# wells-wood-research/timed-design

Measured on AMD Instinct MI355X. Metric: residue_frames_per_sec, higher is better.
Workload: dtype f32

## Files before the change

timed-design_amd/csrc/common.h:

```cpp
#pragma once
#include <hip/hip_runtime.h>
#include <stdint.h>
#include <string>
#include <vector>

#include "../../include/timed_hip.h"

enum : int {
    OP_INPUT = 0, OP_CONV3D, OP_DENSE, OP_BN, OP_ACT, OP_MAXPOOL, OP_AVGPOOL, OP_GAP, OP_GMP,
    OP_FLATTEN, OP_CONCAT, OP_ADD, OP_IDENTITY
};
enum : int { ACT_LINEAR = 0, ACT_RELU, ACT_ELU, ACT_SOFTMAX, ACT_SIGMOID, ACT_TANH, ACT_LEAKY };

void th_set_error(const char* fmt, ...);
#define TH_FAIL(code, ...)          \
    do {                            \
        th_set_error(__VA_ARGS__);  \
        return (code);              \
    } while (0)
#define HIP_TRY(expr)                                                                            \
    do {                                                                                         \
        hipError_t _e = (expr);                                                                  \
        if (_e != hipSuccess) {                                                                  \
            th_set_error("%s failed: %s (%s:%d)", #expr, hipGetErrorString(_e), __FILE__, __LINE__); \
            return TH_EHIP;                                                                      \
        }                                                                                        \
    } while (0)

#ifndef TH_KNOCKOUTS
#define TH_KNOCKOUTS 0
#endif
#if TH_KNOCKOUTS
#define TH_KNOCK_FIELD int dbg;
#define TH_KNOCK(a) ((a).dbg)
#define TH_KNOCK_SET(a, v) ((a).dbg = (v))
#else
#define TH_KNOCK_FIELD
#define TH_KNOCK(a) 0
#define TH_KNOCK_SET(a, v) ((void)0)
#endif

struct ThKnobs {
    int winograd = 1;
    int wino_split = 1;
    int wfused = 1;
    int wf_split = 1;
    int lanes = 1, lane_lag = 1;
    int guard = 1;
    int first_wino = 1;
    int first_split = 1;
    int conv_gl = 1;
    int dense_gemm = 1;
    int first_int = 1;
    int no_pool_first = 0;
    int no_tail_fuse = 0;
    int conv_notail = 0, n16_resident = 0;
    int wf_resident = 0, wf_noblk = 0;
    long long wino_piece = 0;
    int wino_b3var = 2, wino_nomid = 0;
#if TH_KNOCKOUTS
    int wf_dbg = 0, first_dbg = 0, wino_dbg = 0, conv_dbg = 0, pw_dbg = 0;
#endif
    std::string nondefault;
};
int th_knobs_read(ThKnobs* k);
inline const ThKnobs& th_knobs_of(const ThKnobs* k) { static const ThKnobs dflt; return k ? *k : dflt; }

hipError_t th_malloc_retry_impl(void** p, size_t bytes);
template <class T> inline hipError_t th_malloc_retry(T** p, size_t bytes) { return th_malloc_retry_impl(reinterpret_cast<void**>(p), bytes); }

int th_usable_cpus();

struct TView {
    float* p = nullptr;
    int D = 1, H = 1, W = 1, C = 0;
    int cs = 0;
    int coff = 0;
    int64_t fs = 0;
    int blk = 0;
    int V() const { return D * H * W; }
};

#define TH_MAX_POST 4
enum : int { POP_ACT = 1, POP_AFFINE = 2 };
struct PostOps {
    int n = 0;
    int type[TH_MAX_POST] = {0, 0, 0, 0};
    int act[TH_MAX_POST] = {0, 0, 0, 0};
    float alpha[TH_MAX_POST] = {0, 0, 0, 0};
    const float* scale[TH_MAX_POST] = {nullptr, nullptr, nullptr, nullptr};
    const float* shift[TH_MAX_POST] = {nullptr, nullptr, nullptr, nullptr};
    int monotone = 0;
};
struct PreOp {
    const float* scale = nullptr;
    const float* shift = nullptr;
    int act = ACT_LINEAR;
    float alpha = 0.f;
};

struct ConvGeom {
    int kd, kh, kw, sd, sh, sw, dd, dh, dw;
    int pz, py, px;
};
int launch_convert_frames(hipStream_t s, const void* src, int dtype, int64_t n, int V, int C, TView dst);
int launch_conv3d_direct(hipStream_t s, int64_t n, TView in, TView out, ConvGeom g, const float* w, const float* bias,
                         PreOp pre, PostOps post);
int launch_pool3d(hipStream_t s, int64_t n, TView in, TView out, ConvGeom g, int is_max);
int launch_eltwise(hipStream_t s, int64_t n, TView in, TView out, PostOps ops);
int launch_global_pool(hipStream_t s, int64_t n, TView in, TView out, int is_max);
int launch_dense(hipStream_t s, int64_t n, TView in, TView out, const float* w, const float* bias, PostOps post);
inline bool conv_gl_wanted(int knob, const ConvGeom& g, int Vo) { return knob == 2 || (knob == 1 && (g.sd > 1 || g.sh > 1 || g.sw > 1 || Vo <= 64)); }
bool conv_gl_ok(int Cin, int Cout, int in_cs, int in_coff, int64_t in_fs);
size_t conv_gl_wpk_floats(const ConvGeom& g, int Cin, int Cout);
double conv_gl_exec_flops(const ConvGeom& g, int Cin, int Cout, int Vo);
std::string conv_gl_label(int Cout);
void conv_gl_pack_weights(const ConvGeom& g, int Cin, int Cout, const float* w, float* dst);
int launch_conv_gl(hipStream_t s, int64_t n, TView in, TView out, ConvGeom g, int Cin, int Cout, const float* wpk, const float* bias, PreOp pre, PostOps post);
bool dense_gemm_ok(int F, int O, int64_t xfs);
int launch_dense_gemm(hipStream_t s, int64_t n, TView in, TView out, const float* w, const float* bias, PostOps post);
int launch_softmax(hipStream_t s, int64_t n, TView in, TView out);
int launch_gap_softmax(hipStream_t s, int64_t n, TView in, TView logits, TView probs);
int launch_tail_dense(hipStream_t s, int64_t n, TView in, PostOps pre, TView pooled, TView logits, TView probs, const float* w,
                      const float* bias, PostOps post, int softmax);
int launch_copy(hipStream_t s, int64_t n, TView in, TView out);
int launch_add(hipStream_t s, int64_t n, TView a, TView b, TView out);
int launch_synth_frames(hipStream_t s, float* d, int64_t n, int side, int channels, int atoms, uint64_t seed);

struct ConvMfmaPlan {
    int cfg = -1;
    int CI = 0, CS = 0;
    int BN = 0;
    int nnb = 0;
    int nchunks = 0;
    int pool = 0;
    int Dc = 0, Hc = 0, Wc = 0;
    int FB = 1, ZB = 0, nzb = 1;
    int Zp = 0, Hp = 0, Wp = 0;
    int rows_pf = 0;
    size_t lds_bytes = 0;
    size_t tab_off = 0;
    size_t wpk_floats = 0;
// ... 148 lines not shown
```

timed-design_amd/csrc/conv_wino.hip:

```cpp
#include "bf16x3.h"
#include "common.h"
#include "device_math.h"
#include "wino_tables.h"

#include <algorithm>
#include <cstdlib>
#include <cstring>
#include <thread>
#include <vector>

namespace {

constexpr int kZ = WINO_N;
constexpr int kNF = 64;
constexpr int kKC = 32;
constexpr int kCB = 128;

template <int R, int C>
__device__ __forceinline__ void wino_apply(const float (&T)[R][C], const float (&in)[C], float (&out)[R]) {
#pragma unroll
    for (int r = 0; r < R; ++r) {
        float acc = 0.f;
        bool first = true;
#pragma unroll
// ... 92 lines not shown

template <int kP, bool GAP = false>
__global__ void __launch_bounds__(256) k_wino_out(const WinoOutArgs a) {
    constexpr int kPos = kP * kP;
    const unsigned idx = blockIdx.x * 256u + threadIdx.x;
    const unsigned co = idx % (unsigned)a.Cout, f = idx / (unsigned)a.Cout;
    if (f >= (unsigned)a.n) return;
    const unsigned ioff = f * (unsigned)a.Coutp + co;
    const unsigned ooff = f * (unsigned)a.out_fs + co;
    const int64_t pstride = a.Ns * a.Coutp;
    const float bv = a.bias ? a.bias[co] : 0.f;
    const bool elu_bn = a.post.n == 2 && a.post.type[0] == POP_ACT && a.post.act[0] == ACT_ELU && a.post.type[1] == POP_AFFINE;
    const float ealpha = a.post.alpha[0], esc = elu_bn ? a.post.scale[1][co] : 1.f, esh = elu_bn ? a.post.shift[1][co] : 0.f;
    float* __restrict__ out0 = a.out + a.out_coff;
    float gsum = 0.f;
#pragma unroll 1
    for (int z = 0; z < kZ; ++z) {
        float t[kP][kZ];
        const float* __restrict__ pos = a.M + (int64_t)z * kPos * pstride;
#pragma unroll
        for (int aa = 0; aa < kP; ++aa) {
            float m[kP];
#pragma unroll
            for (int b = 0; b < kP; ++b) m[b] = (pos + (int64_t)(aa * kP + b) * pstride)[ioff];
            WinoTab<kP>::inv(m, t[aa]);
        }
        float y[kZ * kZ];
#pragma unroll
        for (int k = 0; k < kZ; ++k) {
            float col[kP], o[kZ];
#pragma unroll
            for (int aa = 0; aa < kP; ++aa) col[aa] = t[aa][k];
            WinoTab<kP>::inv(col, o);
#pragma unroll
            for (int j = 0; j < kZ; ++j) y[j * kZ + k] = o[j] + bv;
        }
        if (elu_bn) {
#pragma unroll
            for (int k = 0; k < kZ * kZ; ++k) y[k] = fmaf(y[k] > 0.f ? y[k] : ealpha * (__expf(y[k]) - 1.f), esc, esh);
        } else
        for (int i = 0; i < a.post.n; ++i) {
            if (a.post.type[i] == POP_AFFINE) {
                const float sc = a.post.scale[i][co], sh = a.post.shift[i][co];
#pragma unroll
                for (int k = 0; k < kZ * kZ; ++k) y[k] = fmaf(y[k], sc, sh);
            } else {
                th_act_vec<kZ * kZ>(y, a.post.act[i], a.post.alpha[i]);
            }
        }
        if (GAP) {
#pragma unroll
            for (int v = 0; v < kZ * kZ; ++v) gsum += y[v];
            continue;
        }
        float* __restrict__ vox = out0 + (int64_t)z * kZ * kZ * a.out_cs;
#pragma unroll
        for (int v = 0; v < kZ * kZ; ++v) (vox + (int64_t)v * a.out_cs)[ooff] = y[v];
    }
    if (GAP) out0[ooff] = gsum / (float)(kZ * kZ * kZ);
}

struct WinoMidArgs {
    const float* M; int64_t Ns; int Coutp;
    int C;
    const float* bias;
    PostOps post;
    float* V;
    int Cn;
    int64_t n;
};

template <int kP>
__global__ void __launch_bounds__(256) k_wino_mid(const WinoMidArgs a) {
    constexpr int kPos = kP * kP;
    const unsigned idx = blockIdx.x * 256u + threadIdx.x;
    const unsigned c = idx % (unsigned)a.Cn, f = idx / (unsigned)a.Cn;
    if (f >= (unsigned)a.n) return;
    const unsigned ioff = f * (unsigned)a.Coutp + c;
    const unsigned ooff = f * (unsigned)a.Cn + c;
    const int64_t ipstride = a.Ns * a.Coutp, opstride = a.Ns * a.Cn;
    if (c >= (unsigned)a.C) {
        for (int z = 0; z < kZ; ++z) {
            float* __restrict__ opos = a.V + (int64_t)z * kPos * opstride;
            for (int q = 0; q < kPos; ++q) (opos + (int64_t)q * opstride)[ooff] = 0.f;
        }
        return;
    }
    const float bv = a.bias ? a.bias[c] : 0.f;
    const bool elu_bn = a.post.n == 2 && a.post.type[0] == POP_ACT && a.post.act[0] == ACT_ELU && a.post.type[1] == POP_AFFINE;
    const float ealpha = a.post.alpha[0], esc = elu_bn ? a.post.scale[1][c] : 1.f, esh = elu_bn ? a.post.shift[1][c] : 0.f;
#pragma unroll 1
    for (int z = 0; z < kZ; ++z) {
        float t[kP][kZ];
        const float* __restrict__ ipos = a.M + (int64_t)z * kPos * ipstride;
#pragma unroll
        for (int aa = 0; aa < kP; ++aa) {
            float m[kP];
#pragma unroll
            for (int b = 0; b < kP; ++b) m[b] = (ipos + (int64_t)(aa * kP + b) * ipstride)[ioff];
            WinoTab<kP>::inv(m, t[aa]);
        }
        float y[kZ * kZ];
#pragma unroll
        for (int k = 0; k < kZ; ++k) {
            float col[kP], o[kZ];
#pragma unroll
            for (int aa = 0; aa < kP; ++aa) col[aa] = t[aa][k];
            WinoTab<kP>::inv(col, o);
#pragma unroll
            for (int j = 0; j < kZ; ++j) y[j * kZ + k] = o[j] + bv;
        }
        if (elu_bn) {
#pragma unroll
            for (int k = 0; k < kZ * kZ; ++k) y[k] = fmaf(y[k] > 0.f ? y[k] : ealpha * (__expf(y[k]) - 1.f), esc, esh);
        } else
        for (int i = 0; i < a.post.n; ++i) {
            if (a.post.type[i] == POP_AFFINE) {
                const float sc = a.post.scale[i][c], sh = a.post.shift[i][c];
#pragma unroll
                for (int k = 0; k < kZ * kZ; ++k) y[k] = fmaf(y[k], sc, sh);
            } else {
                th_act_vec<kZ * kZ>(y, a.post.act[i], a.post.alpha[i]);
            }
        }
        float u[kP][kZ];
#pragma unroll
        for (int k = 0; k < kZ; ++k) {
            float col[kZ], o[kP];
#pragma unroll
            for (int j = 0; j < kZ; ++j) col[j] = y[j * kZ + k];
            WinoTab<kP>::fwd(col, o);
#pragma unroll
            for (int aa = 0; aa < kP; ++aa) u[aa][k] = o[aa];
        }
        float* __restrict__ opos = a.V + (int64_t)z * kPos * opstride;
#pragma unroll
        for (int aa = 0; aa < kP; ++aa) {
            float o[kP];
            WinoTab<kP>::fwd(u[aa], o);
#pragma unroll
            for (int b = 0; b < kP; ++b) (opos + (int64_t)(aa * kP + b) * opstride)[ooff] = o[b];
        }
    }
}

struct WinoGemmArgs {
    const float* V; const float* U; float* M;
    int64_t Ns;
    int Cin, Coutp;
    int Cout;
    int nfb, ncb;
    int npos;
    unsigned total;
    unsigned per_xcd;
    TH_KNOCK_FIELD
};

__device__ __forceinline__ constexpr bool wino_tap_ok(int zi, int dz) { return zi - dz + 1 >= 0 && zi - dz + 1 < kZ; }

struct WinoTile {
    unsigned p, fb, cb;
    int lane, wave;
    bool active;
};

__device__ __forceinline__ bool wino_tile_index(const WinoGemmArgs& a, unsigned& L) {
    const unsigned xcd = blockIdx.x & 7u, slot = blockIdx.x >> 3;
    L = xcd * a.per_xcd + slot;
    return slot < a.per_xcd && L < a.total;
}
__device__ __forceinline__ WinoTile wino_tile(const WinoGemmArgs& a, unsigned L) {
    WinoTile t;
    t.cb = L % (unsigned)a.ncb;
    t.fb = (L / (unsigned)a.ncb) % (unsigned)a.nfb;
    t.p = L / (unsigned)(a.ncb * a.nfb);
    t.lane = threadIdx.x & 63;
    t.wave = __builtin_amdgcn_readfirstlane(threadIdx.x >> 6);
    t.active = (int)(t.cb * kCB) + t.wave * 32 < a.Cout;
    return t;
}

__global__ void __launch_bounds__(256, 2) k_wino_gemm(const WinoGemmArgs a) {
    __shared__ __attribute__((aligned(16))) float lds[kZ * kNF * kKC];
    unsigned L;
    if (!wino_tile_index(a, L)) return;
    const WinoTile t = wino_tile(a, L);
    const unsigned p = t.p, fb = t.fb, cb = t.cb;
    const int lane = t.lane, wave = t.wave;
    const int j = lane & 31, h = lane >> 5;
    const int nchunks = a.Cin / kKC;
    const int S = a.Cin / 8;
    const float4* wq = reinterpret_cast<const float4*>(a.U) + ((size_t)((p * a.ncb + cb) * 4 + wave) * S * 3) * 64 + lane;
    const float* vbase = a.V + ((int64_t)p * a.Ns + (int64_t)fb * kNF) * a.Cin;
    const int64_t zstride = (int64_t)a.npos * a.Ns * a.Cin;

    f32x16 acc[kZ][2];
#pragma unroll
    for (int z = 0; z < kZ; ++z)
#pragma unroll
        for (int rt = 0; rt < 2; ++rt)
#pragma unroll
            for (int r = 0; r < 16; ++r) acc[z][rt][r] = 0.f;

    float4 bw[2][3];
#pragma unroll
    for (int dz = 0; dz < 3; ++dz) bw[0][dz] = wq[dz * 64];
    const int r0 = 8 * wave + (lane >> 3);
    const float* gsrc = vbase + (int64_t)r0 * a.Cin + (((lane & 7) ^ (lane >> 3)) << 2);
    const int64_t rstride32 = (int64_t)32 * a.Cin;
    unsigned aoff[kKC / 8];
#pragma unroll
    for (int s = 0; s < kKC / 8; ++s) aoff[s] = (unsigned)(j * kKC + (((2 * s + h) ^ (j & 7)) << 2));
    constexpr int kSlots = kKC / 8;
    static_assert(kSlots % 2 == 0, "the weight register sets alternate per k-slot");

    for (int ch = 0; ch < nchunks; ++ch) {
        __syncthreads();
        if (!(TH_KNOCK(a) & 1))
#pragma unroll
        for (int i = 0; i < 10; ++i)
            __builtin_amdgcn_global_load_lds(gsrc + (i >> 1) * zstride + (i & 1) * rstride32 + ch * kKC,
                                             lds + (size_t)(i * 4 + wave) * 256, 16, 0, 0);
        __syncthreads();
        if (!t.active) continue;
// ... 234 lines not shown
#pragma unroll
    for (int z = 0; z < kZ; ++z) vrsrc[z] = __builtin_amdgcn_make_buffer_rsrc(const_cast<float*>(vbase + z * zstride), 0, 0xffffffffu, 0x00020000);
    const int r0 = 8 * t.wave + (lane >> 3), g4 = lane & 7;
    const unsigned goff = (unsigned)(r0 * a.Cin + 4 * g4) * 4u;
    const unsigned rstride32_b = (unsigned)(32 * a.Cin * 4);
    unsigned char* const sdst = lds + r0 * 64 + (((g4 >> 1) ^ ((r0 >> 2) & 3)) << 4) + ((g4 & 1) << 3);
    const unsigned char* aptr[2];
#pragma unroll
    for (int ks = 0; ks < 2; ++ks) aptr[ks] = lds + j * 64 + (((2 * ks + h) ^ ((j >> 2) & 3)) << 4);

    for (int ch = 0; ch < nchunks; ++ch) {
        __syncthreads();
        wino_stage_split(a, vrsrc, goff, rstride32_b, ch, sdst);
        __syncthreads();
        if (!t.active) continue;
#pragma unroll
        for (int st = 0; st < 6; ++st) {
            const int ks = st / 3, dz = st % 3, cur = st & 1;
            {
                const int sg = ch * 6 + st;
                const int nx = sg + 1 < S ? sg + 1 : sg;
                if (TH_KNOCK(a) & 4) {
#pragma unroll
                    for (int pc = 0; pc < 3; ++pc) bw[cur ^ 1][pc] = bw[cur][pc];
                } else
#pragma unroll
                for (int pc = 0; pc < 3; ++pc) bw[cur ^ 1][pc] = wq[(size_t)(nx * 3 + pc) * 64];
            }
            bf16x8 bf[3];
#pragma unroll
            for (int pc = 0; pc < 3; ++pc) bf[pc] = __builtin_bit_cast(bf16x8, bw[cur][pc]);
            const int nzi = 5 - (dz != 1), z0 = dz == 2 ? 1 : 0;
#pragma unroll
            for (int k = 0; k < kZ; ++k) {
                if (k >= nzi) continue;
                const int zi = z0 + k, zo = zi - dz + 1;
                bf16x8 af[2][3];
#pragma unroll
                for (int rt = 0; rt < 2; ++rt)
#pragma unroll
                    for (int pc = 0; pc < 3; ++pc)
                        af[rt][pc] = __builtin_bit_cast(bf16x8, *reinterpret_cast<const uint4*>(aptr[ks] + pc * kB3Slab + (zi * kNF + rt * 32) * 64));
#pragma unroll
                for (int c = 0; c < 6; ++c)
#pragma unroll
                    for (int rt = 0; rt < 2; ++rt)
                        acc[zo][rt] = __builtin_amdgcn_mfma_f32_32x32x16_bf16(af[rt][kWinoPA[c]], bf[kWinoPB[c]], acc[zo][rt], 0, 0, 0);
                __builtin_amdgcn_sched_barrier(0);
            }
        }
    }
    if (!t.active) return;
    if (TH_KNOCK(a) & 2) {
        float sum = 0.f;
#pragma unroll
        for (int z = 0; z < kZ; ++z)
#pragma unroll
            for (int rt = 0; rt < 2; ++rt)
#pragma unroll
                for (int r = 0; r < 16; ++r) sum += acc[z][rt][r];
        if (sum == 12345.678f) a.M[0] = sum;
        return;
    }
    __syncthreads();
    float* T = reinterpret_cast<float*>(lds) + t.wave * (32 * 36);
    const int rr = lane >> 3, c4 = (lane & 7) * 4;
    float* mb = a.M + ((int64_t)t.p * a.Ns + (int64_t)t.fb * kNF) * a.Coutp + t.cb * kCB + t.wave * 32 + c4;
    const int64_t mz = (int64_t)a.npos * a.Ns * a.Coutp;
#pragma unroll
    for (int z = 0; z < kZ; ++z)
#pragma unroll
        for (int rt = 0; rt < 2; ++rt) {
#pragma unroll
            for (int r = 0; r < 16; ++r) T[((r & 3) + 8 * (r >> 2) + 4 * h) * 36 + j] = acc[z][rt][r];
#pragma unroll
            for (int k = 0; k < 4; ++k) {
                const int row = rr + 8 * k;
                *reinterpret_cast<float4*>(mb + z * mz + (int64_t)(rt * 32 + row) * a.Coutp) = *reinterpret_cast<const float4*>(T + row * 36 + c4);
            }
        }
}


__global__ void __launch_bounds__(256, 2) k_wino_gemm_n32(const WinoGemmArgs a) {
    __shared__ __attribute__((aligned(16))) float4 tile[4][32 * 8];
    const int tid = threadIdx.x, lane = tid & 63;
    const int wave = __builtin_amdgcn_readfirstlane(tid >> 6);
    const int j = lane & 31, h = lane >> 5;
    const int nfb32 = (int)(a.Ns / 32);
    const int groups = (nfb32 + 3) / 4;
    const unsigned p = blockIdx.x / (unsigned)groups;
    const int fb = (int)(blockIdx.x % (unsigned)groups) * 4 + wave;
    if (fb >= nfb32) return;
    const int nchunks = a.Cin / kKC;
    const uint4* wq = reinterpret_cast<const uint4*>(a.U) + (size_t)p * nchunks * 18 * 64 + lane;
    const float* vbase = a.V + ((int64_t)p * a.Ns + (int64_t)fb * 32) * a.Cin;
    const int64_t zstride = (int64_t)a.npos * a.Ns * a.Cin;
    __amdgpu_buffer_rsrc_t vrsrc[kZ];
#pragma unroll
    for (int z = 0; z < kZ; ++z) vrsrc[z] = __builtin_amdgcn_make_buffer_rsrc(const_cast<float*>(vbase + z * zstride), 0, 0xffffffffu, 0x00020000);
    const int lr = lane >> 3, lg = lane & 7;
    const unsigned goff = (unsigned)(lr * a.Cin + 4 * lg) * 4u;
    const unsigned row8_b = (unsigned)(8 * a.Cin * 4);
    float4* const T = tile[wave];

    f32x16 acc[kZ];
#pragma unroll
    for (int z = 0; z < kZ; ++z)
#pragma unroll
        for (int r = 0; r < 16; ++r) acc[z][r] = 0.f;

    auto load_plane = [&](float4 (&x)[4], int ch, int zi) {
#pragma unroll
        for (int k = 0; k < 4; ++k)
            x[k] = __builtin_bit_cast(float4, __builtin_amdgcn_raw_buffer_load_b128(vrsrc[zi], goff, k * row8_b + ch * (kKC * 4), 0));
    };
    auto transpose = [&](const float4 (&x)[4], float4 (&f)[4]) {
#pragma unroll
        for (int k = 0; k < 4; ++k) { const int r = 8 * k + lr; T[r * 8 + (lg ^ ((r >> 1) & 7))] = x[k]; }
#pragma unroll
        for (int g = 0; g < 4; ++g) f[g] = T[j * 8 + ((4 * h + g) ^ ((j >> 1) & 7))];
    };
    auto split8 = [&](const float4& lo, const float4& hi, bf16x8 (&f)[3]) {
        const float v[8] = {lo.x, lo.y, lo.z, lo.w, hi.x, hi.y, hi.z, hi.w};
        unsigned hw[4], mw[4], lw[4];
#pragma unroll
        for (int q = 0; q < 4; ++q) bf16x3::split(v[2 * q], v[2 * q + 1], hw[q], mw[q], lw[q]);
        f[0] = __builtin_bit_cast(bf16x8, make_uint4(hw[0], hw[1], hw[2], hw[3]));
        f[1] = __builtin_bit_cast(bf16x8, make_uint4(mw[0], mw[1], mw[2], mw[3]));
        f[2] = __builtin_bit_cast(bf16x8, make_uint4(lw[0], lw[1], lw[2], lw[3]));
    };

    float4 xs[3][4];
    auto load_step = [&](float4 (&x)[4], int step_ch, int zi) {
        load_plane(x, step_ch < nchunks ? step_ch : nchunks - 1, zi);
    };
    load_step(xs[0], 0, 0);
    load_step(xs[1], 0, 1);
    for (int ch0 = 0; ch0 < nchunks; ch0 += 3) {
#pragma unroll
        for (int cc = 0; cc < 3; ++cc) {
            const int ch = ch0 + cc;
            if (ch >= nchunks) break;
            uint4 bw[2][3][3];
#pragma unroll
            for (int ks = 0; ks < 2; ++ks)
#pragma unroll
                for (int dz = 0; dz < 3; ++dz)
#pragma unroll
                    for (int pc = 0; pc < 3; ++pc) bw[ks][dz][pc] = wq[(size_t)(((ch * 2 + ks) * 3 + dz) * 3 + pc) * 64];
#pragma unroll
            for (int zi = 0; zi < kZ; ++zi) {
                const int t = cc * kZ + zi;
                float4 fr[4];
                transpose(xs[t % 3], fr);
                {
                    const int t2 = t + 2, c2 = ch0 + t2 / kZ, z2 = t2 % kZ;
                    load_step(xs[t2 % 3], c2, z2);
                }
                bf16x8 af[2][3];
                split8(fr[0], fr[1], af[0]);
                split8(fr[2], fr[3], af[1]);
#pragma unroll
                for (int q = 0; q < 6; ++q)
#pragma unroll
                    for (int ks = 0; ks < 2; ++ks)
#pragma unroll
                        for (int dz = 0; dz < 3; ++dz) {
                            if (!wino_tap_ok(zi, dz)) continue;
                            acc[zi - dz + 1] = __builtin_amdgcn_mfma_f32_32x32x16_bf16(af[ks][kWinoPA[q]], __builtin_bit_cast(bf16x8, bw[ks][dz][kWinoPB[q]]),
                                                                                       acc[zi - dz + 1], 0, 0, 0);
                        }
                __builtin_amdgcn_sched_barrier(0);
            }
        }
    }
    float* mb = a.M + ((int64_t)p * a.Ns + (int64_t)fb * 32) * a.Coutp + j;
    const int64_t mz = (int64_t)a.npos * a.Ns * a.Coutp;
#pragma unroll
    for (int z = 0; z < kZ; ++z)
#pragma unroll
        for (int r = 0; r < 16; ++r) mb[z * mz + (int64_t)((r & 3) + 8 * (r >> 2) + 4 * h) * a.Coutp] = acc[z][r];
}

}

bool conv_wino_plan(const TView& in, const TView& out, const ConvGeom& g, int Cin, int Cout, int scheme, int split, const ThKnobs& kn, ConvWinoPlan* p) {
    if (g.kd != 3 || g.kh != 3 || g.kw != 3 || g.sd != 1 || g.sh != 1 || g.sw != 1 || g.dd != 1 || g.dh != 1 || g.dw != 1) return false;
    if (g.pz != 1 || g.py != 1 || g.px != 1) return false;
    if (in.D != kZ || in.H != kZ || in.W != kZ || out.D != kZ || out.H != kZ || out.W != kZ) return false;
    const bool narrow = split && Cout <= 32 && Cin >= 128;
    if (Cin < kKC || (Cout < 64 && !narrow)) return false;
    if (scheme != 9 && scheme != 7) return false;
    const int kPos = scheme * scheme;
    p->P = scheme;
    p->Cin = Cin; p->Cout = Cout;
    p->Cinp = (Cin + kKC - 1) / kKC * kKC;
    const int Cinp = p->Cinp;
    p->narrow = narrow ? 1 : 0;
    p->Coutp = narrow ? 32 : (Cout + kCB - 1) / kCB * kCB;
    p->ncb = narrow ? 1 : p->Coutp / kCB;
    p->split = split ? 1 : 0;
    p->b3var = split && !narrow ? kn.wino_b3var : 0;
    p->knobs = &kn;
    p->wpk_floats = (size_t)kPos * 3 * Cinp * p->Coutp * (p->split ? 3 : 2) / 2;
    p->v_fpf = (int64_t)kZ * kPos * Cinp;
    p->m_fpf = (int64_t)kZ * kPos * p->Coutp;
    p->gemm_flops = 2.0 * kPos * 13 * Cin * (double)Cout;
    p->exec_flops = 2.0 * kPos * 13 * Cinp * (double)((Cout + 31) / 32 * 32);
    p->label = std::string("conv_wino<") + (scheme == 9 ? "F(3,3)+F(2,3)" : "F(5,3)") + " in-plane, z direct; gemm " + (narrow ? "32f x 32" : "64f x " + std::to_string(kCB)) + "c, K" + std::to_string(Cinp) + (Cinp != Cin ? " (" + std::to_string(Cin) + " real)" : "") +
               (p->split ? "; bf16x3 split operands, 6 products, fp32 accumulate" : "") + ">";
    return true;
}

void conv_wino_pack_weights(const ConvWinoPlan& p, const float* w, float* dst) {
    const int Cin = p.Cin, Cinp = p.Cinp, Cout = p.Cout, S = Cinp / 8, ncb = p.ncb, kP = p.P;
    auto G = [kP](int a, int j) { return kP == 9 ? kWinoG9[a][j] : kWinoG7[a][j]; };
    std::memset(dst, 0, p.wpk_floats * sizeof(float));
    auto work = [&](int ci_lo, int ci_hi) {
        std::vector<double> t((size_t)kP * 3 * Cout), u((size_t)Cout);
        for (int ci = ci_lo; ci < ci_hi; ++ci) {
            const int s = ci / 8, hh = (ci % 8) / 4, tt = ci % 4;
            for (int dz = 0; dz < 3; ++dz) {
                for (int a = 0; a < kP; ++a)
                    for (int k = 0; k < 3; ++k) {
                        double* tr = &t[((size_t)a * 3 + k) * Cout];
                        std::fill(tr, tr + Cout, 0.0);
                        for (int jj = 0; jj < 3; ++jj) {
                            const double g = G(a, jj);
                            if (g == 0.0) continue;
                            const float* wr = w + ((((size_t)dz * 3 + jj) * 3 + k) * Cin + ci) * Cout;
                            for (int co = 0; co < Cout; ++co) tr[co] += g * (double)wr[co];
                        }
                    }
                for (int a = 0; a < kP; ++a)
                    for (int b = 0; b < kP; ++b) {
                        std::fill(u.begin(), u.end(), 0.0);
                        for (int k = 0; k < 3; ++k) {
                            const double g = G(b, k);
                            if (g == 0.0) continue;
                            const double* tr = &t[((size_t)a * 3 + k) * Cout];
                            for (int co = 0; co < Cout; ++co) u[co] += g * tr[co];
                        }
                        const int pos = a * kP + b;
                        if (p.narrow) {
                            uint16_t* d16 = reinterpret_cast<uint16_t*>(dst);
                            const int chunk = ci / kKC, h16 = (ci % kKC) / 16, ks = (ci % 16) / 8, e = ci % 8, nch = Cinp / kKC;
                            for (int co = 0; co < Cout; ++co) {
                                uint16_t pc[3];
                                bf16x3::split3(u[co], pc);
                                const size_t frag = ((size_t)(pos * nch + chunk) * 2 + ks) * 3 + dz;
                                for (int q = 0; q < 3; ++q) d16[((frag * 3 + q) * 64 + (h16 * 32 + co)) * 8 + e] = pc[q];
                            }
                            continue;
                        }
                        if (p.split && p.b3var == 2) {
                            uint16_t* d16 = reinterpret_cast<uint16_t*>(dst);
                            const int chunk = ci / kKC, g8 = (ci % kKC) / 8, e = ci % 8, nch = Cinp / kKC;
                            for (int co = 0; co < Cout; ++co) {
                                const int cb = co / kCB, wv = (co % kCB) / 32, ct = (co % 32) / 16, c = co % 16;
                                uint16_t pc[3];
                                bf16x3::split3(u[co], pc);
                                const size_t frag = ((size_t)(((pos * ncb + cb) * 4 + wv) * nch + chunk) * 2 + ct) * 3 + dz;
                                for (int q = 0; q < 3; ++q) d16[((frag * 3 + q) * 64 + (g8 * 16 + c)) * 8 + e] = pc[q];
                            }
                            continue;
                        }
                        if (p.split) {
                            uint16_t* d16 = reinterpret_cast<uint16_t*>(dst);
                            const int chunk = ci / kKC, ks = (ci % kKC) / 16, h8 = (ci % 16) / 8, e = ci % 8, nsteps = (Cinp / kKC) * 6;
                            for (int co = 0; co < Cout; ++co) {
                                const int cb = co / kCB, wv = (co % kCB) / 32, j = co % 32;
                                uint16_t pc[3];
                                bf16x3::split3(u[co], pc);
                                const size_t step = (size_t)((pos * ncb + cb) * 4 + wv) * nsteps + (size_t)(chunk * 2 + ks) * 3 + dz;
                                for (int q = 0; q < 3; ++q) d16[((step * 3 + q) * 64 + (h8 * 32 + j)) * 8 + e] = pc[q];
                            }
                            continue;
                        }
                        for (int co = 0; co < Cout; ++co) {
                            const int cb = co / kCB, wv = (co % kCB) / 32, j = co % 32;
                            dst[((((size_t)(pos * ncb + cb) * 4 + wv) * S + s) * 3 + dz) * 256 + (hh * 32 + j) * 4 + tt] = (float)u[co];
                        }
                    }
            }
        }
    };
    const int nt = std::max(1, std::min({th_usable_cpus(), 32, Cin / 8}));
    if (nt == 1) { work(0, Cin); return; }
    std::vector<std::thread> th;
    for (int k = 0; k < nt; ++k) th.emplace_back(work, (int)((int64_t)Cin * k / nt), (int)((int64_t)Cin * (k + 1) / nt));
    for (auto& x : th) x.join();
}

static int64_t wino_piece(const ConvWinoPlan& p, int64_t n, int64_t Ns, int64_t fs, int width) {
    const int64_t lim = (1ll << 31) - 1;
    if (Ns * width > lim) return 0;
    const int64_t forced = th_knobs_of(p.knobs).wino_piece;
    const int64_t piece = std::max<int64_t>(1, std::min<int64_t>(n, lim / std::max<int64_t>(fs, 1)));
    return forced > 0 ? std::min(piece, forced) : piece;
}

int launch_wino_in(hipStream_t s, int64_t n, const ConvWinoPlan& p, TView in, float* V, PreOp pre) {
    if (n <= 0) return TH_OK;
    const int64_t Ns = (n + kNF - 1) / kNF * kNF;
    const int64_t piece = wino_piece(p, n, Ns, in.fs, p.Cinp);
    if (!piece) TH_FAIL(TH_EUNSUP, "conv_wino: %lld frames per launch exceed the 32-bit offsets of the transform kernels", (long long)n);
    const bool has_pre = pre.scale || pre.act != ACT_LINEAR;
    for (int64_t f0 = 0; f0 < n; f0 += piece) {
        const int64_t cnt = std::min(piece, n - f0);
        WinoInArgs ia;
        ia.in = in.p + f0 * in.fs; ia.in_fs = in.fs; ia.in_cs = in.cs; ia.in_coff = in.coff; ia.Cin = p.Cinp; ia.Creal = p.Cin; ia.pre = pre;
        ia.V = V + f0 * p.Cinp; ia.Ns = Ns; ia.n = cnt;
        const dim3 grid((unsigned)((cnt * p.Cinp + 255) / 256));
        if (p.P == 9) {
            if (has_pre) hipLaunchKernelGGL((k_wino_in<true, 9>), grid, dim3(256), 0, s, ia);
            else hipLaunchKernelGGL((k_wino_in<false, 9>), grid, dim3(256), 0, s, ia);
        } else {
            if (has_pre) hipLaunchKernelGGL((k_wino_in<true, 7>), grid, dim3(256), 0, s, ia);
            else hipLaunchKernelGGL((k_wino_in<false, 7>), grid, dim3(256), 0, s, ia);
        }
    }
    HIP_TRY(hipGetLastError());
    return TH_OK;
}

int launch_wino_gemm(hipStream_t s, int64_t n, const ConvWinoPlan& p, const float* V, float* M, const float* wpk) {
    if (n <= 0) return TH_OK;
    WinoGemmArgs ga;
    ga.V = V; ga.U = wpk; ga.M = M; ga.Ns = (n + kNF - 1) / kNF * kNF; ga.Cin = p.Cinp; ga.Coutp = p.Coutp;
    ga.Cout = p.Cout;
    ga.nfb = (int)(ga.Ns / kNF); ga.ncb = p.ncb;
    ga.npos = p.P * p.P;
    ga.total = (unsigned)(ga.npos * ga.nfb * ga.ncb);
    ga.per_xcd = (ga.total + 7) / 8;
    TH_KNOCK_SET(ga, th_knobs_of(p.knobs).wino_dbg);
    if (p.narrow) {
        const int64_t groups = (ga.Ns / 32 + 3) / 4;
        hipLaunchKernelGGL(k_wino_gemm_n32, dim3((unsigned)(ga.npos * groups)), dim3(256), 0, s, ga);
    } else if (p.split) {
        if (p.b3var == 2) hipLaunchKernelGGL(k_wino_gemm_b3_16, dim3(ga.per_xcd * 8), dim3(256), 0, s, ga);
        else hipLaunchKernelGGL(k_wino_gemm_b3_32, dim3(ga.per_xcd * 8), dim3(256), 0, s, ga);
    }
    else hipLaunchKernelGGL(k_wino_gemm, dim3(ga.per_xcd * 8), dim3(256), 0, s, ga);
    HIP_TRY(hipGetLastError());
    return TH_OK;
}

int launch_wino_out(hipStream_t s, int64_t n, const ConvWinoPlan& p, const float* M, TView out, const float* bias, PostOps post, bool gap) {
    if (n <= 0) return TH_OK;
    const int64_t Ns = (n + kNF - 1) / kNF * kNF;
    const int64_t piece = wino_piece(p, n, Ns, out.fs, p.Coutp);
    if (!piece) TH_FAIL(TH_EUNSUP, "conv_wino: %lld frames per launch exceed the 32-bit offsets of the transform kernels", (long long)n);
    for (int64_t f0 = 0; f0 < n; f0 += piece) {
        const int64_t cnt = std::min(piece, n - f0);
        WinoOutArgs oa;
        oa.M = M + f0 * p.Coutp; oa.Ns = Ns; oa.Coutp = p.Coutp; oa.Cout = p.Cout; oa.bias = bias; oa.post = post;
        oa.out = out.p + f0 * out.fs; oa.out_fs = out.fs; oa.out_cs = out.cs; oa.out_coff = out.coff; oa.n = cnt;
        const dim3 grid((unsigned)((cnt * p.Cout + 255) / 256));
        if (gap) {
            if (p.P == 9) hipLaunchKernelGGL((k_wino_out<9, true>), grid, dim3(256), 0, s, oa);
            else hipLaunchKernelGGL((k_wino_out<7, true>), grid, dim3(256), 0, s, oa);
        } else if (p.P == 9) hipLaunchKernelGGL(k_wino_out<9>, grid, dim3(256), 0, s, oa);
        else hipLaunchKernelGGL(k_wino_out<7>, grid, dim3(256), 0, s, oa);
    }
    HIP_TRY(hipGetLastError());
    return TH_OK;
}

int launch_wino_mid(hipStream_t s, int64_t n, const ConvWinoPlan& p, const float* M, float* V_next, const float* bias, PostOps post) {
    if (n <= 0) return TH_OK;
    const int64_t Ns = (n + kNF - 1) / kNF * kNF;
    if (Ns * (int64_t)p.Coutp >= (1ll << 31))
        TH_FAIL(TH_EUNSUP, "conv_wino: %lld frames per launch exceed the 32-bit offsets of the transform kernels", (long long)n);
    const int Cn = (p.Cout + kKC - 1) / kKC * kKC;
    if (Ns * (int64_t)Cn >= (1ll << 31))
        TH_FAIL(TH_EUNSUP, "conv_wino: %lld frames per launch exceed the 32-bit offsets of the transform kernels", (long long)n);
    WinoMidArgs ma;
    ma.M = M; ma.Ns = Ns; ma.Coutp = p.Coutp; ma.C = p.Cout; ma.Cn = Cn; ma.bias = bias; ma.post = post; ma.V = V_next; ma.n = n;
    const dim3 grid((unsigned)((n * (int64_t)Cn + 255) / 256));
    if (p.P == 9) hipLaunchKernelGGL(k_wino_mid<9>, grid, dim3(256), 0, s, ma);
    else hipLaunchKernelGGL(k_wino_mid<7>, grid, dim3(256), 0, s, ma);
    HIP_TRY(hipGetLastError());
    return TH_OK;
}
```

timed-design_amd/csrc/runtime.hip:

```cpp
#include "model.h"

#include <chrono>
#include <cstdarg>
#include <cstdio>
#include <cstring>

using namespace th_rt;

static thread_local char g_err[1024] = "";
void th_set_error(const char* fmt, ...) {
    va_list ap;
    va_start(ap, fmt);
    vsnprintf(g_err, sizeof g_err, fmt, ap);
    va_end(ap);
}

int th_knobs_read(ThKnobs* k) {
    *k = ThKnobs();
    std::string& nd = k->nondefault;
    auto note = [&](const char* name, const char* v) { nd += (nd.empty() ? "" : " "); nd += name; nd += "="; nd += v; };
    auto num = [&](const char* name, int* dst, int lo, int hi) {
        const char* e = getenv(name);
        if (!e) return;
        const int v = std::max(lo, std::min(hi, atoi(e)));
        if (v != *dst) note(name, e);
        *dst = v;
    };
    auto flag = [&](const char* name, int* dst) {
        const char* e = getenv(name);
        if (e && *e && atoi(e) != 0) { *dst = 1; note(name, e); }
    };
    const char* refused = nullptr;
#if TH_KNOCKOUTS
#define KNOCK(name, field) num(name, &k->field, 0, 1 << 20)
#else
    auto refuse = [&](const char* name) { const char* e = getenv(name); if (!refused && e && atoi(e) != 0) refused = name; };
#define KNOCK(name, field) refuse(name)
#endif
    num("TH_WINOGRAD", &k->winograd, 0, 2);
    num("TH_WINO_SPLIT", &k->wino_split, 0, 1);
    num("TH_WFUSED", &k->wfused, 0, 1);
    num("TH_WF_SPLIT", &k->wf_split, 0, 1);
    if (const char* e = getenv("TH_LANES")) { k->lanes = atoi(e) == 2 ? 2 : 1; if (k->lanes != 1) note("TH_LANES", e); }
    num("TH_LANE_LAG", &k->lane_lag, 0, 1 << 20);
    num("TH_GUARD", &k->guard, 0, 2);
    num("TH_FIRST_WINO", &k->first_wino, 0, 1);
    num("TH_FIRST_SPLIT", &k->first_split, 0, 1);
    num("TH_FIRST_INT", &k->first_int, 0, 1);
    num("TH_DENSE_GEMM", &k->dense_gemm, 0, 1);
    num("TH_CONV_GL", &k->conv_gl, 0, 2);
    KNOCK("TH_FIRST_DBG", first_dbg);
    flag("TH_NO_POOL_FIRST", &k->no_pool_first);
    flag("TH_NO_TAIL_FUSE", &k->no_tail_fuse);
    flag("TH_CONV_NOTAIL", &k->conv_notail);
    KNOCK("TH_CONV_DBG", conv_dbg);
    num("TH_N16_RESIDENT", &k->n16_resident, 0, 1 << 20);
    KNOCK("TH_PW_DBG", pw_dbg);
    num("TH_WF_RESIDENT", &k->wf_resident, 0, 1 << 20);
    KNOCK("TH_WF_DBG", wf_dbg);
    num("TH_WF_NOBLK", &k->wf_noblk, 0, 1);
    if (const char* e = getenv("TH_WINO_PIECE")) { k->wino_piece = std::max(0ll, atoll(e)); if (k->wino_piece) note("TH_WINO_PIECE", e); }
    KNOCK("TH_WINO_DBG", wino_dbg);
    num("TH_WINO_B3VAR", &k->wino_b3var, 0, 2);
    num("TH_WINO_NOMID", &k->wino_nomid, 0, 1);
#undef KNOCK
    if (refused)
        TH_FAIL(TH_EINVAL, "%s is set, but this library has no timing knock-outs: build the knock-out library "
                           "(tools/build_knockouts.py) and load it through TIMED_HIP_LIB", refused);
    return TH_OK;
}

int th_rt::load_common(th_model* m, const ThKnobs& knobs) {
    HIP_TRY(hipSetDevice(m->device));
    HIP_TRY(hipDeviceGetAttribute(&m->ncu, hipDeviceAttributeMultiprocessorCount, m->device));
    HIP_TRY(hipStreamCreateWithFlags(&m->stream, hipStreamNonBlocking));
    HIP_TRY(hipStreamCreateWithFlags(&m->pipe.copy_stream, hipStreamNonBlocking));
    HIP_TRY(hipStreamCreateWithFlags(&m->pipe.d2h_stream, hipStreamNonBlocking));
    HIP_TRY(hipStreamCreateWithFlags(&m->lane.stream2, hipStreamNonBlocking));
    HIP_TRY(hipEventCreateWithFlags(&m->lane.ev_fork, hipEventDisableTiming));
    HIP_TRY(hipEventCreateWithFlags(&m->lane.ev_join, hipEventDisableTiming));
    m->knobs = knobs;
    m->lane.lanes = m->knobs.lanes; m->lane.lag = m->knobs.lane_lag;
    for (int r = 0; r < th_model::kRing; ++r) {
        HIP_TRY(hipEventCreateWithFlags(&m->pipe.ev_h2d[r], hipEventDisableTiming));
        HIP_TRY(hipEventCreateWithFlags(&m->pipe.ev_free[r], hipEventDisableTiming));
    }
    for (th_model::Ticket& t : m->pipe.tickets) {
        HIP_TRY(hipEventCreateWithFlags(&t.computed, hipEventDisableTiming));
        HIP_TRY(hipEventCreateWithFlags(&t.done, hipEventDisableTiming));
    }
    int rc = parse_pack(m);
    if (rc) return rc;
    return plan(m);
}

th_model::~th_model() {
    (void)hipSetDevice(device);
    if (stream) (void)hipStreamSynchronize(stream);
    if (pipe.copy_stream) (void)hipStreamSynchronize(pipe.copy_stream);
    if (pipe.d2h_stream) (void)hipStreamSynchronize(pipe.d2h_stream);
    if (lane.stream2) (void)hipStreamSynchronize(lane.stream2);
    for (float* p : dev_allocs) cached_free(p);
    for (Buffer& b : bufs) if (b.dev) cached_free(b.dev);
    for (int r = 0; r < th_model::kRing; ++r) {
        if (pipe.d_in_ring[r]) cached_free(pipe.d_in_ring[r]);
        if (pipe.d_sp_ring[r]) cached_free(pipe.d_sp_ring[r]);
        if (pipe.ev_h2d[r]) (void)hipEventDestroy(pipe.ev_h2d[r]);
        if (pipe.ev_free[r]) (void)hipEventDestroy(pipe.ev_free[r]);
    }
    for (th_model::Ticket& t : pipe.tickets) {
        if (t.d_out) cached_free(t.d_out);
        if (t.h_out) (void)hipHostFree(t.h_out);
        if (t.computed) (void)hipEventDestroy(t.computed);
        if (t.done) (void)hipEventDestroy(t.done);
    }
    if (lane.stream2) (void)hipStreamDestroy(lane.stream2);
    if (lane.ev_fork) (void)hipEventDestroy(lane.ev_fork);
    if (lane.ev_join) (void)hipEventDestroy(lane.ev_join);
    if (pipe.copy_stream) (void)hipStreamDestroy(pipe.copy_stream);
    if (pipe.d2h_stream) (void)hipStreamDestroy(pipe.d2h_stream);
    for (hipEvent_t e : ev_pool) (void)hipEventDestroy(e);
    if (stream) (void)hipStreamDestroy(stream);
}

extern "C" {

int th_version(void) { return 1; }
const char* th_last_error(void) { return g_err; }

int th_device_count(int* n_out) {
    if (!n_out) TH_FAIL(TH_EINVAL, "null argument");
    int n = 0;
    hipError_t e = hipGetDeviceCount(&n);
    if (e != hipSuccess) { *n_out = 0; TH_FAIL(TH_EHIP, "hipGetDeviceCount: %s", hipGetErrorString(e)); }
    *n_out = n;
    return TH_OK;
}

int th_device_info(int device, char* name, size_t name_len, char* arch, size_t arch_len, int* cus) {
    hipDeviceProp_t p;
    HIP_TRY(hipGetDeviceProperties(&p, device));
    if (name && name_len) snprintf(name, name_len, "%s", p.name);
    if (arch && arch_len) snprintf(arch, arch_len, "%s", p.gcnArchName);
    if (cus) *cus = p.multiProcessorCount;
    return TH_OK;
}

// ... 181 lines not shown
```

Measured before the change: 587,700.

## Stream Winograd n32 GEMM input through a direct global-to-LDS DMA ring

The narrow Winograd GEMM kernel stops loading input planes into registers and then writing them to LDS for the transpose. It now issues global_load_lds_dwordx4 through inline asm into a ring of DEPTH LDS slots (default 2, selectable by knob), waiting on vmcnt before reading each slot. This is meant to cut register pressure and VGPR-to-LDS store traffic and to overlap loads with MFMA work, at the cost of more LDS per block and fragile hand-written m0/waitcnt handling. Separately, the mid transform kernel switches its loads and stores to nontemporal hints to avoid polluting the cache.

Result: no change. 593,600, median of 2 (+1.0%).

```diff
diff --git a/timed-design_amd/csrc/common.h b/timed-design_amd/csrc/common.h
--- a/timed-design_amd/csrc/common.h
+++ b/timed-design_amd/csrc/common.h
@@ -58,6 +58,7 @@
     int wf_resident = 0, wf_noblk = 0;
     long long wino_piece = 0;
     int wino_b3var = 2, wino_nomid = 0;
+    int wino_n32_depth = 2;
 #if TH_KNOCKOUTS
     int wf_dbg = 0, first_dbg = 0, wino_dbg = 0, conv_dbg = 0, pw_dbg = 0;
 #endif
diff --git a/timed-design_amd/csrc/conv_wino.hip b/timed-design_amd/csrc/conv_wino.hip
--- a/timed-design_amd/csrc/conv_wino.hip
+++ b/timed-design_amd/csrc/conv_wino.hip
@@ -198,7 +198,7 @@
     if (c >= (unsigned)a.C) {
         for (int z = 0; z < kZ; ++z) {
             float* __restrict__ opos = a.V + (int64_t)z * kPos * opstride;
-            for (int q = 0; q < kPos; ++q) (opos + (int64_t)q * opstride)[ooff] = 0.f;
+            for (int q = 0; q < kPos; ++q) __builtin_nontemporal_store(0.f, opos + (int64_t)q * opstride + ooff);
         }
         return;
     }
@@ -213,7 +213,7 @@
         for (int aa = 0; aa < kP; ++aa) {
             float m[kP];
 #pragma unroll
-            for (int b = 0; b < kP; ++b) m[b] = (ipos + (int64_t)(aa * kP + b) * ipstride)[ioff];
+            for (int b = 0; b < kP; ++b) m[b] = __builtin_nontemporal_load(ipos + (int64_t)(aa * kP + b) * ipstride + ioff);
             WinoTab<kP>::inv(m, t[aa]);
         }
         float y[kZ * kZ];
@@ -255,7 +255,7 @@
             float o[kP];
             WinoTab<kP>::fwd(u[aa], o);
 #pragma unroll
-            for (int b = 0; b < kP; ++b) (opos + (int64_t)(aa * kP + b) * opstride)[ooff] = o[b];
+            for (int b = 0; b < kP; ++b) __builtin_nontemporal_store(o[b], opos + (int64_t)(aa * kP + b) * opstride + ooff);
         }
     }
 }
@@ -656,8 +656,18 @@
 }
 
 
+__device__ __forceinline__ void wino_glds(const void* base, unsigned voff, unsigned lds_dst) {
+    unsigned keep;
+    asm volatile("s_mov_b32 %0, m0\n\ts_mov_b32 m0, %3\n\ts_nop 0\n\tglobal_load_lds_dwordx4 %1, %2\n\ts_mov_b32 m0, %0"
+                 : "=&s"(keep) : "v"(voff), "s"(base), "s"(lds_dst) : "memory");
+}
+template <int N> __device__ __forceinline__ void wino_dma_wait() { asm volatile("s_waitcnt vmcnt(%0)" :: "n"(N) : "memory"); }
+__device__ __forceinline__ void wino_lds_wait() { asm volatile("s_waitcnt lgkmcnt(0)" ::: "memory"); }
+
+template <int DEPTH>
 __global__ void __launch_bounds__(256, 2) k_wino_gemm_n32(const WinoGemmArgs a) {
-    __shared__ __attribute__((aligned(16))) float4 tile[4][32 * 8];
+    static_assert(DEPTH >= 1 && 4 * (DEPTH - 1) <= 63, "the ring's wait is one vmcnt immediate");
+    __shared__ __attribute__((aligned(16))) float4 tile[4][DEPTH][32 * 8];
     const int tid = threadIdx.x, lane = tid & 63;
     const int wave = __builtin_amdgcn_readfirstlane(tid >> 6);
     const int j = lane & 31, h = lane >> 5;
@@ -670,13 +680,13 @@
     const uint4* wq = reinterpret_cast<const uint4*>(a.U) + (size_t)p * nchunks * 18 * 64 + lane;
     const float* vbase = a.V + ((int64_t)p * a.Ns + (int64_t)fb * 32) * a.Cin;
     const int64_t zstride = (int64_t)a.npos * a.Ns * a.Cin;
-    __amdgpu_buffer_rsrc_t vrsrc[kZ];
-#pragma unroll
-    for (int z = 0; z < kZ; ++z) vrsrc[z] = __builtin_amdgcn_make_buffer_rsrc(const_cast<float*>(vbase + z * zstride), 0, 0xffffffffu, 0x00020000);
     const int lr = lane >> 3, lg = lane & 7;
-    const unsigned goff = (unsigned)(lr * a.Cin + 4 * lg) * 4u;
-    const unsigned row8_b = (unsigned)(8 * a.Cin * 4);
-    float4* const T = tile[wave];
+    unsigned voff[4];
+#pragma unroll
+    for (int k = 0; k < 4; ++k) { const int r = 8 * k + lr; voff[k] = (unsigned)(r * a.Cin + 4 * (lg ^ ((r >> 1) & 7))) * 4u; }
+    const float4* const T = tile[wave][0];
+    const unsigned tbase = (unsigned)(uintptr_t)T;
+    const int nsteps = nchunks * kZ;
 
     f32x16 acc[kZ];
 #pragma unroll
@@ -684,16 +694,10 @@
 #pragma unroll
         for (int r = 0; r < 16; ++r) acc[z][r] = 0.f;
 
-    auto load_plane = [&](float4 (&x)[4], int ch, int zi) {
-#pragma unroll
-        for (int k = 0; k < 4; ++k)
-            x[k] = __builtin_bit_cast(float4, __builtin_amdgcn_raw_buffer_load_b128(vrsrc[zi], goff, k * row8_b + ch * (kKC * 4), 0));
-    };
-    auto transpose = [&](const float4 (&x)[4], float4 (&f)[4]) {
-#pragma unroll
-        for (int k = 0; k < 4; ++k) { const int r = 8 * k + lr; T[r * 8 + (lg ^ ((r >> 1) & 7))] = x[k]; }
-#pragma unroll
-        for (int g = 0; g < 4; ++g) f[g] = T[j * 8 + ((4 * h + g) ^ ((j >> 1) & 7))];
+    auto issue = [&](int ch, int zi, int slot) {
+        const float* src = vbase + zi * zstride + ch * kKC;
+#pragma unroll
+        for (int k = 0; k < 4; ++k) wino_glds(src, voff[k], tbase + (unsigned)(slot * 4096 + k * 1024));
     };
     auto split8 = [&](const float4& lo, const float4& hi, bf16x8 (&f)[3]) {
         const float v[8] = {lo.x, lo.y, lo.z, lo.w, hi.x, hi.y, hi.z, hi.w};
@@ -705,48 +709,44 @@
         f[2] = __builtin_bit_cast(bf16x8, make_uint4(lw[0], lw[1], lw[2], lw[3]));
     };
 
-    float4 xs[3][4];
-    auto load_step = [&](float4 (&x)[4], int step_ch, int zi) {
-        load_plane(x, step_ch < nchunks ? step_ch : nchunks - 1, zi);
-    };
-    load_step(xs[0], 0, 0);
-    load_step(xs[1], 0, 1);
-    for (int ch0 = 0; ch0 < nchunks; ch0 += 3) {
-#pragma unroll
-        for (int cc = 0; cc < 3; ++cc) {
-            const int ch = ch0 + cc;
-            if (ch >= nchunks) break;
-            uint4 bw[2][3][3];
-#pragma unroll
-            for (int ks = 0; ks < 2; ++ks)
-#pragma unroll
-                for (int dz = 0; dz < 3; ++dz)
-#pragma unroll
-                    for (int pc = 0; pc < 3; ++pc) bw[ks][dz][pc] = wq[(size_t)(((ch * 2 + ks) * 3 + dz) * 3 + pc) * 64];
-#pragma unroll
-            for (int zi = 0; zi < kZ; ++zi) {
-                const int t = cc * kZ + zi;
-                float4 fr[4];
-                transpose(xs[t % 3], fr);
-                {
-                    const int t2 = t + 2, c2 = ch0 + t2 / kZ, z2 = t2 % kZ;
-                    load_step(xs[t2 % 3], c2, z2);
-                }
-                bf16x8 af[2][3];
-                split8(fr[0], fr[1], af[0]);
-                split8(fr[2], fr[3], af[1]);
-#pragma unroll
-                for (int q = 0; q < 6; ++q)
-#pragma unroll
-                    for (int ks = 0; ks < 2; ++ks)
-#pragma unroll
-                        for (int dz = 0; dz < 3; ++dz) {
-                            if (!wino_tap_ok(zi, dz)) continue;
-                            acc[zi - dz + 1] = __builtin_amdgcn_mfma_f32_32x32x16_bf16(af[ks][kWinoPA[q]], __builtin_bit_cast(bf16x8, bw[ks][dz][kWinoPB[q]]),
-                                                                                       acc[zi - dz + 1], 0, 0, 0);
-                        }
-                __builtin_amdgcn_sched_barrier(0);
-            }
+#pragma unroll
+    for (int d = 0; d < DEPTH; ++d)
+        if (d < nsteps) issue(d / kZ, d % kZ, d);
+    int slot = 0;
+    for (int ch = 0; ch < nchunks; ++ch) {
+        uint4 bw[2][3][3];
+#pragma unroll
+        for (int ks = 0; ks < 2; ++ks)
+#pragma unroll
+            for (int dz = 0; dz < 3; ++dz)
+#pragma unroll
+                for (int pc = 0; pc < 3; ++pc) bw[ks][dz][pc] = wq[(size_t)(((ch * 2 + ks) * 3 + dz) * 3 + pc) * 64];
+#pragma unroll
+        for (int zi = 0; zi < kZ; ++zi) {
+            const int t = ch * kZ + zi;
+            if (t + DEPTH - 1 < nsteps) wino_dma_wait<4 * (DEPTH - 1)>();
+            else wino_dma_wait<0>();
+            float4 fr[4];
+            const float4* Ts = T + slot * 256;
+#pragma unroll
+            for (int g = 0; g < 4; ++g) fr[g] = Ts[j * 8 + ((4 * h + g) ^ ((j >> 1) & 7))];
+            wino_lds_wait();
+            if (t + DEPTH < nsteps) issue(ch + (zi + DEPTH) / kZ, (zi + DEPTH) % kZ, slot);
+            slot = slot + 1 == DEPTH ? 0 : slot + 1;
+            bf16x8 af[2][3];
+            split8(fr[0], fr[1], af[0]);
+            split8(fr[2], fr[3], af[1]);
+#pragma unroll
+            for (int q = 0; q < 6; ++q)
+#pragma unroll
+                for (int ks = 0; ks < 2; ++ks)
+#pragma unroll
+                    for (int dz = 0; dz < 3; ++dz) {
+                        if (!wino_tap_ok(zi, dz)) continue;
+                        acc[zi - dz + 1] = __builtin_amdgcn_mfma_f32_32x32x16_bf16(af[ks][kWinoPA[q]], __builtin_bit_cast(bf16x8, bw[ks][dz][kWinoPB[q]]),
+                                                                                   acc[zi - dz + 1], 0, 0, 0);
+                    }
+            __builtin_amdgcn_sched_barrier(0);
         }
     }
     float* mb = a.M + ((int64_t)p * a.Ns + (int64_t)fb * 32) * a.Coutp + j;
@@ -911,7 +911,13 @@
     TH_KNOCK_SET(ga, th_knobs_of(p.knobs).wino_dbg);
     if (p.narrow) {
         const int64_t groups = (ga.Ns / 32 + 3) / 4;
-        hipLaunchKernelGGL(k_wino_gemm_n32, dim3((unsigned)(ga.npos * groups)), dim3(256), 0, s, ga);
+        const dim3 grid((unsigned)(ga.npos * groups));
+        switch (th_knobs_of(p.knobs).wino_n32_depth) {
+            case 1: hipLaunchKernelGGL((k_wino_gemm_n32<1>), grid, dim3(256), 0, s, ga); break;
+            case 3: hipLaunchKernelGGL((k_wino_gemm_n32<3>), grid, dim3(256), 0, s, ga); break;
+            case 4: hipLaunchKernelGGL((k_wino_gemm_n32<4>), grid, dim3(256), 0, s, ga); break;
+            default: hipLaunchKernelGGL((k_wino_gemm_n32<2>), grid, dim3(256), 0, s, ga); break;
+        }
     } else if (p.split) {
         if (p.b3var == 2) hipLaunchKernelGGL(k_wino_gemm_b3_16, dim3(ga.per_xcd * 8), dim3(256), 0, s, ga);
         else hipLaunchKernelGGL(k_wino_gemm_b3_32, dim3(ga.per_xcd * 8), dim3(256), 0, s, ga);
diff --git a/timed-design_amd/csrc/runtime.hip b/timed-design_amd/csrc/runtime.hip
--- a/timed-design_amd/csrc/runtime.hip
+++ b/timed-design_amd/csrc/runtime.hip
@@ -63,6 +63,7 @@
     KNOCK("TH_WINO_DBG", wino_dbg);
     num("TH_WINO_B3VAR", &k->wino_b3var, 0, 2);
     num("TH_WINO_NOMID", &k->wino_nomid, 0, 1);
+    num("TH_WINO_N32_DEPTH", &k->wino_n32_depth, 1, 4);
 #undef KNOCK
     if (refused)
         TH_FAIL(TH_EINVAL, "%s is set, but this library has no timing knock-outs: build the knock-out library "
```
